# utiasASRL/mm_masking

Measured on AMD Instinct MI355X. Metric: scan-pairs/s (mask-CNN + 10-iter dICP fwd+bwd), higher is better.
Workload: dtype bf16; 1 GPU; BASELINE configs[2]: train_icp_weights step fwd+bwd, batch=32 per GPU, 10 dICP iters, point-to-plane Huber, dim=2; 400x3360 polar radar -> GO-CFAR + peaks + polar->Cartesian 640x640 -> U-Net (hand-written NHWC bf16 MFMA kernels, fp32 masters) -> dICP (fp32 points, fp64 normal equations) -> rot+trans+mask_pts loss -> Adam; batch_per_gpu=32, global_batch=32, scan_pts_pad=5120, map_pts=20000, map_pts_pad=20480, icp_iters=10, parallelism=dp1, scene_density=survey (SURVEY.md 8d: 3 500-5 000 valid scan points of 5 120)

## Files before the change

### include/mmk.h

```cpp
#ifndef MMK_H_
#define MMK_H_

#include <stddef.h>
#include <stdint.h>

#ifdef __cplusplus
extern "C" {
#endif

#define MMK_VERSION 502

#define MMK_OK 0
#define MMK_ERR_ARG (-1)
#define MMK_ERR_HIP (-2)
#define MMK_ERR_WORKSPACE (-3)

#define MMK_ICP_PT2PT 0
#define MMK_ICP_PT2PL 1

#define MMK_NN_BRUTE 0
#define MMK_NN_GRID 1

#define MMK_LOSS_NONE 0
#define MMK_LOSS_CAUCHY 1
// ... 167 lines not shown
                              const float *grad_out, float *grad_x, void *stream);


int mmk_cfar_mask(const float *raw, int32_t B, int32_t A, int32_t R, int32_t w2,
                  int32_t guard, int32_t mincol, int32_t maxcol, float a_thresh,
                  float b_thresh, int32_t diff, float steep_fact, float *mask,
                  void *stream);

int mmk_cfar_mask_bwd(const float *raw, const float *grad_mask , int32_t B, int32_t A, int32_t R, int32_t w2,
                      int32_t guard, int32_t mincol, int32_t maxcol, float a_thresh, float b_thresh, float steep_fact,
                      float *grad_raw , void *stream);

int mmk_cfar_mask_p(const float *raw, int32_t B, int32_t A, int32_t R, int32_t w2, int32_t guard, int32_t mincol,
                    int32_t maxcol, const float *a_thresh, const float *b_thresh, int32_t per_scan, int32_t diff,
                    float steep_fact, float *mask, void *stream);

size_t mmk_cfar_mask_bwd_p_ws_bytes(int32_t B, int32_t A);
int mmk_cfar_mask_bwd_p(const float *raw, const float *grad_mask , int32_t B, int32_t A, int32_t R, int32_t w2,
                        int32_t guard, int32_t mincol, int32_t maxcol, const float *a_thresh, const float *b_thresh,
                        int32_t per_scan, float steep_fact, float *grad_raw , float *grad_a,
                        float *grad_b , void *workspace, size_t workspace_bytes, void *stream);

size_t mmk_extract_peaks_workspace_bytes(int32_t B, int32_t A, int32_t R, int32_t max_pts);
int mmk_extract_peaks(const float *mask, int32_t B, int32_t A, int32_t R, float res,
                      const float *azimuths , const float *times ,
                      const float *T_ab, int32_t diff, float steep_fact, int32_t max_pts,
                      float *out_pc, int32_t *out_count, void *workspace,
                      size_t workspace_bytes, void *stream);
int mmk_extract_peaks_t(const float *mask, int32_t B, int32_t A, int32_t R, float res,
                        const float *azimuths , const float *times ,
                        const float *T_ab, int32_t diff, float steep_fact, int32_t max_pts,
                        float *out_pc, int32_t *out_count, void *workspace,
                        size_t workspace_bytes, float *out_time , void *stream);
size_t mmk_extract_peaks_bwd_workspace_bytes(int32_t B, int32_t A, int32_t R, int32_t max_pts);
int mmk_extract_peaks_bwd(const float *mask, int32_t B, int32_t A, int32_t R, float res, const float *azimuths ,
                          const float *T_ab, int32_t diff, float steep_fact, int32_t max_pts,
                          const float *grad_pc , float *grad_mask , void *workspace,
                          size_t workspace_bytes, void *stream);

int mmk_deskew_points(const float *pc , const float *t , const float *twist ,
                      int32_t B, int32_t N, float *out , void *stream);
size_t mmk_deskew_points_bwd_workspace_bytes(int32_t B, int32_t N);
int mmk_deskew_points_bwd(const float *pc , const float *t , const float *twist ,
                          int32_t B, int32_t N, const float *grad_out ,
                          float *grad_pc , float *grad_twist ,
                          void *workspace, size_t workspace_bytes, void *stream);

int mmk_polar_to_cart(const float *polar, const float *azimuths ,
                      const float *range_grid, const float *angle_grid, int32_t B,
                      int32_t A, int32_t R, int32_t W, float radar_resolution,
                      int32_t interpolate_crossover, int32_t fix_wobble, float *cart,
                      void *stream);
int mmk_polar_to_cart_pair(const float *polar, const float *polar2, const float *azimuths,
                           const float *range_grid, const float *angle_grid, int32_t B, int32_t A,
                           int32_t R, int32_t W, float radar_resolution, int32_t interpolate_crossover,
                           int32_t fix_wobble, float *cart, float *cart2, void *stream);

int mmk_cart_to_polar(const double *cart, const double *sin_az, const double *cos_az, const double *range_coords,
                      int32_t B, int32_t A, int32_t R, int32_t H, int32_t W, double cart_resolution, double *polar,
                      void *stream);

size_t mmk_polar_to_cart_bwd_ws_bytes(int32_t B, int32_t A, int32_t R, int32_t W);
int mmk_polar_to_cart_bwd(const float *grad_cart , const float *azimuths , const float *range_grid,
                          const float *angle_grid, int32_t B, int32_t A, int32_t R, int32_t W, float radar_resolution,
                          int32_t interpolate_crossover, int32_t fix_wobble, float *grad_polar , void *ws,
                          size_t ws_bytes, void *stream);
// ... 200 lines not shown
```

### mm_masking_amd/csrc/mmk_radar.hip

```cpp
#include <math.h>

#include "mmk_common.h"

namespace {

constexpr int RT = 256;

template <int NTHR = RT>
__device__ __forceinline__ double block_excl_scan(double v, double *sm, double *total)
{
    const int lane = threadIdx.x & 63, wv = threadIdx.x >> 6;
    double inc = v;
#pragma unroll
    for (int off = 1; off < 64; off <<= 1) {
        double o = __shfl_up(inc, off, 64);
        if (lane >= off) inc += o;
    }
    if (lane == 63) sm[wv] = inc;
    __syncthreads();
    double base = 0.0, tot = 0.0;
#pragma unroll
    for (int w = 0; w < NTHR / 64; ++w) {
        if (w < wv) base += sm[w];
        tot += sm[w];
    }
    __syncthreads();
    *total = tot;
    return base + inc - v;
}

__device__ __forceinline__ int block_excl_scan_i(int v, int *sm, int *total)
{
    const int lane = threadIdx.x & 63, wv = threadIdx.x >> 6;
    int inc = v;
#pragma unroll
    for (int off = 1; off < 64; off <<= 1) {
        int o = __shfl_up(inc, off, 64);
        if (lane >= off) inc += o;
    }
    if (lane == 63) sm[wv] = inc;
    __syncthreads();
    int base = 0, tot = 0;
#pragma unroll
    for (int w = 0; w < RT / 64; ++w) {
        if (w < wv) base += sm[w];
        tot += sm[w];
    }
    __syncthreads();
    *total = tot;
    return base + inc - v;
}

constexpr int CFAR_T = 512;

struct CfarThVal {
    static constexpr bool per_row = false, params = false;
    float a, b;
    __device__ __forceinline__ int scan_of(int) const { return 0; }
    __device__ __forceinline__ float a_of(int) const { return a; }
    __device__ __forceinline__ float b_of(int) const { return b; }
};
struct CfarThPtr {
    static constexpr bool per_row = true, params = true;
    const float *a, *b;
    int stride, A;
    double *part;
    __device__ __forceinline__ int scan_of(int row) const { return row / A; }
    __device__ __forceinline__ float a_of(int scan) const { return a[scan * stride]; }
    __device__ __forceinline__ float b_of(int scan) const { return b[scan * stride]; }
};

template <class TH>
__global__ __launch_bounds__(CFAR_T) void cfar_mask_kernel(const float *__restrict__ raw, int R, int w2, int guard,
                                                       int mincol, int maxcol, TH thr, int diff,
                                                       float steep, float *__restrict__ mask)
{
    const float a_th = thr.a_of(blockIdx.y), b_th = thr.b_of(blockIdx.y);
    extern __shared__ __attribute__((aligned(16))) unsigned char smem[];
    double *cs = reinterpret_cast<double *>(smem);
    float *row = reinterpret_cast<float *>(cs + (R + 1));
    __shared__ double wsum[CFAR_T / 64];
// ... 168 lines not shown
    }
    if (threadIdx.x == 0) total[b] = tot;
}

__global__ __launch_bounds__(RT) void peaks_emit_kernel(const float *__restrict__ mask, int R, float res, int diff,
                                                        float steep, const int32_t *__restrict__ row_off, int cap,
                                                        float *__restrict__ mval, int32_t *__restrict__ mrow_out)
{
    extern __shared__ __attribute__((aligned(16))) float lrow_dyn[];
    __shared__ int sm[RT / 64];
    const int a = blockIdx.x, b = blockIdx.y, A = gridDim.x;
    const int rowid = b * A + a;
    const float *mrow = stage_row(mask + (size_t)rowid * R, R, lrow_dyn);
    const int L = (R - 1 + RT - 1) / RT;
    const int j0 = min(R - 1, (int)threadIdx.x * L), j1 = min(R - 1, j0 + L);
    int cnt = 0;
    for (int j = j0; j < j1; ++j) cnt += (peak_value(mrow, j, R, res, diff, steep) != 0.0f) ? 1 : 0;
    int tot;
    int g = row_off[rowid] + block_excl_scan_i(cnt, sm, &tot);
    if (cnt != 0) {
        for (int j = j0; j < j1; ++j) {
            const float v = peak_value(mrow, j, R, res, diff, steep);
            if (v != 0.0f) {
                if (g < cap) {
                    mval[(size_t)b * cap + g] = v;
                    mrow_out[(size_t)b * cap + g] = a;
                }
                ++g;
            }
        }
    }
}

__global__ void peaks_pair_kernel(const float *__restrict__ mval, const int32_t *__restrict__ mrow, int cap,
                                  const int32_t *__restrict__ total, const float *__restrict__ az,
                                  const float *__restrict__ T_ab, int A, int max_pts, float *__restrict__ out_pc,
                                  int32_t *__restrict__ out_count)
{
    const int k = blockIdx.x * blockDim.x + threadIdx.x;
    const int b = blockIdx.y;
    const int npts = total[b] / 2;
    if (k == 0) out_count[b] = npts;
    if (k >= max_pts) return;
    float x = 0.f, y = 0.f, z = 0.f;
    if (k < npts && 2 * k + 1 < cap) {
        const size_t m = (size_t)b * cap + 2 * k;
        const float rho = (mval[m + 1] + mval[m]) / 2.0f;
        const float phi = (az[b * A + mrow[m + 1]] + az[b * A + mrow[m]]) / 2.0f;
        x = rho * cosf(phi);
        y = rho * sinf(phi);
        if (T_ab) {
            const float *T = T_ab + (size_t)b * 16;
            const float xx = ((T[0] * x + T[1] * y) + T[2] * z) + T[3];
            const float yy = ((T[4] * x + T[5] * y) + T[6] * z) + T[7];
            const float zz = ((T[8] * x + T[9] * y) + T[10] * z) + T[11];
            x = xx; y = yy; z = zz;
        }
    }
    float *o = out_pc + ((size_t)b * max_pts + k) * 3;
    o[0] = x; o[1] = y; o[2] = z;
}

__global__ void peaks_time_kernel(const int32_t *__restrict__ mrow, int cap, const int32_t *__restrict__ total,
                                  const float *__restrict__ times, int A, int max_pts, float *__restrict__ out_time)
{
    const int k = blockIdx.x * blockDim.x + threadIdx.x;
    const int b = blockIdx.y;
    if (k >= max_pts) return;
    const int npts = total[b] / 2;
    float tv = 0.f;
    if (k < npts && 2 * k + 1 < cap) {
        const size_t m = (size_t)b * cap + 2 * k;
        tv = (times[b * A + mrow[m + 1]] + times[b * A + mrow[m]]) / 2.0f;
    }
    out_time[(size_t)b * max_pts + k] = tv;
}

struct D3 {
    double x, y, z;
};
__device__ __forceinline__ D3 cross3(const D3 &a, const D3 &b) { return {a.y * b.z - a.z * b.y, a.z * b.x - a.x * b.z, a.x * b.y - a.y * b.x}; }
__device__ __forceinline__ double dot3(const D3 &a, const D3 &b) { return (a.x * b.x + a.y * b.y) + a.z * b.z; }
__device__ __forceinline__ D3 scale3(double s, const D3 &a) { return {s * a.x, s * a.y, s * a.z}; }
__device__ __forceinline__ D3 add3(const D3 &a, const D3 &b) { return {a.x + b.x, a.y + b.y, a.z + b.z}; }

constexpr double DESKEW_SERIES_CUT = 1e-4;
constexpr int DESKEW_T = 256;

template <bool WITH_D>
__device__ __forceinline__ void deskew_coef(double th2, double &A, double &B, double &C, double &dA, double &dB, double &dC)
{
    if (th2 < DESKEW_SERIES_CUT) {
        const double th4 = th2 * th2, th6 = th4 * th2;
        A = ((1.0 - th2 / 6.0) + th4 / 120.0) - th6 / 5040.0;
        B = ((0.5 - th2 / 24.0) + th4 / 720.0) - th6 / 40320.0;
        C = ((1.0 / 6.0 - th2 / 120.0) + th4 / 5040.0) - th6 / 362880.0;
        if (WITH_D) {
            dA = (-1.0 / 6.0 + th2 / 60.0) - th4 / 1680.0;
            dB = (-1.0 / 24.0 + th2 / 360.0) - th4 / 13440.0;
            dC = (-1.0 / 120.0 + th2 / 2520.0) - th4 / 120960.0;
        }
    } else {
        const double th = sqrt(th2), s = sin(th), c = cos(th);
        A = s / th;
        B = (1.0 - c) / th2;
        C = (th - s) / (th2 * th);
        if (WITH_D) {
            dA = (C - B) * 0.5;
// ... 194 lines not shown
        const float a3 = laz[c3], a2 = laz[c2];
        const float df = ang - a3;
        const float delta = ((df * ((df < 0.f) ? 1.f : 0.f)) * ((c3 > 0) ? 1.f : 0.f)) / ((a3 - a2) + 1e-14f);
        v = (float)c3 + delta;
        dv = (df < 0.f && c3 > 0) ? 1.0f / ((a3 - a2) + 1e-14f) : 0.f;
    } else {
        const float step = (laz[A - 1] - laz[0]) / (float)(A - 1);
        v = (ang - laz[0]) / step;
        dv = 1.0f / step;
    }
    if (u < 0.f) u = 0.f;
    const int rows = wrap ? A + 2 : A;
    if (wrap) v = v + 1.0f;
    const float gx = u / (float)(R - 1) * 2.0f - 1.0f;
    const float gy = v / (float)(rows - 1) * 2.0f - 1.0f;
    const float ix = ((gx + 1.0f) / 2.0f) * (float)(R - 1);
    const float iy = ((gy + 1.0f) / 2.0f) * (float)(rows - 1);
    const float x0 = floorf(ix), y0 = floorf(iy);
    PolarTaps t;
    t.wx = ix - x0;
    t.wy = iy - y0;
    t.xi = (int)x0;
    t.yi = (int)y0;
    return t;
}

__device__ __forceinline__ PolarTaps polar_taps(const float *laz, float rng, float ang, int A, int R, float res, float half_res,
                                                int wrap, int fix_wobble)
{
    float du, dv;
    return polar_taps_slopes(laz, rng, ang, A, R, res, half_res, wrap, fix_wobble, du, dv);
}

__global__ __launch_bounds__(256) void polar_to_cart_kernel(const float *__restrict__ polar,
                                                            const float *__restrict__ az,
                                                            const float *__restrict__ rgrid,
                                                            const float *__restrict__ agrid, int A, int R, int W,
                                                            float res, float half_res, int wrap, int fix_wobble,
                                                            float *__restrict__ cart, const float *__restrict__ polar2,
                                                            float *__restrict__ cart2)
{
    extern __shared__ float laz[];
    const int b = blockIdx.y;
    for (int i = threadIdx.x; i < A; i += blockDim.x) laz[i] = az[(size_t)b * A + i];
    __syncthreads();
    const int tiles_x = (W + 31) >> 5;
    const int px = (blockIdx.x % tiles_x) * 32 + (threadIdx.x & 31), py = (blockIdx.x / tiles_x) * 8 + (threadIdx.x >> 5);
    if (px >= W || py >= W) return;
    const int pix = py * W + px;
    const int rows = wrap ? A + 2 : A;
    const PolarTaps t = polar_taps(laz, rgrid[pix], agrid[pix], A, R, res, half_res, wrap, fix_wobble);
    const int xi = t.xi, yi = t.yi;
    const float wx = t.wx, wy = t.wy;
    const float ex = 1.0f - wx, sy = 1.0f - wy;
    typedef float f32x2u __attribute__((ext_vector_type(2), aligned(4)));
    const int xa = min(max(xi, 0), R - 2);
    const bool shifted = xi > xa;
    int roff[2];
    bool okr[2];
#pragma unroll
    for (int k = 0; k < 2; ++k) {
        const int yk = yi + k;
        okr[k] = !(yk < 0 || yk >= rows);
        int r = yk;
        if (wrap) r = (yk == 0) ? (A - 1) : ((yk == A + 1) ? 0 : yk - 1);
        roff[k] = min(max(r, 0), A - 1) * R + xa;
    }
    const bool okx0 = xi >= 0 && xi < R, okx1 = xi + 1 >= 0 && xi + 1 < R;
    const float *img = polar + (size_t)b * A * R;
    const float *img2 = polar2 != nullptr ? polar2 + (size_t)b * A * R : img;
    f32x2u p1[2], p2[2];
#pragma unroll
    for (int k = 0; k < 2; ++k) p1[k] = *reinterpret_cast<const f32x2u *>(img + roff[k]);
#pragma unroll
    for (int k = 0; k < 2; ++k) p2[k] = *reinterpret_cast<const f32x2u *>(img2 + roff[k]);
    float t1[4], t2[4];
#pragma unroll
    for (int k = 0; k < 2; ++k) {
        t1[2 * k] = (okr[k] && okx0) ? (shifted ? p1[k].y : p1[k].x) : 0.0f;
        t1[2 * k + 1] = (okr[k] && okx1) ? p1[k].y : 0.0f;
        t2[2 * k] = (okr[k] && okx0) ? (shifted ? p2[k].y : p2[k].x) : 0.0f;
        t2[2 * k + 1] = (okr[k] && okx1) ? p2[k].y : 0.0f;
    }
    cart[(size_t)b * W * W + pix] = t1[0] * (sy * ex) + t1[1] * (sy * wx) + t1[2] * (wy * ex) + t1[3] * (wy * wx);
    if (polar2 != nullptr) cart2[(size_t)b * W * W + pix] = t2[0] * (sy * ex) + t2[1] * (sy * wx) + t2[2] * (wy * ex) + t2[3] * (wy * wx);
}

struct Taps {
    int xi, yi;
    float w00, w01, w10, w11;
    float wx, wy;
};

__device__ __forceinline__ Taps weight_taps(const float *__restrict__ p, int H, int W, int cw, float cres)
{
    const float x = p[0], y = p[1];
    const bool fake = (x == 0.0f) && (y == 0.0f);
    const float gu = -x / cres;
    const float gv = y / cres;
    float gx = gv / (float)(cw - 1) * 2.0f;
    float gy = gu / (float)(cw - 1) * 2.0f;
    if (fake) {
        gx = -100.0f;
        gy = -100.0f;
    }
    const float ix = ((gx + 1.0f) / 2.0f) * (float)(W - 1);
    const float iy = ((gy + 1.0f) / 2.0f) * (float)(H - 1);
    const float x0 = floorf(ix), y0 = floorf(iy);
    const float wx = ix - x0, wy = iy - y0;
    Taps t;
    t.xi = (int)x0;
    t.yi = (int)y0;
    t.w00 = (1.0f - wy) * (1.0f - wx);
    t.w01 = (1.0f - wy) * wx;
    t.w10 = wy * (1.0f - wx);
    t.w11 = wy * wx;
    t.wx = wx;
    t.wy = wy;
// ... 929 lines not shown
    if (int rc = check_workspace(who, workspace, workspace_bytes, w.bytes)) return rc;
    hipStream_t st = (hipStream_t)stream;
    if (int rc = launch_peaks_placement(who, mask, B, A, R, res, diff, steep_fact, w, st)) return rc;
    hipLaunchKernelGGL(peaks_pair_kernel, dim3((max_pts + 255) / 256, B), dim3(256), 0, st, w.mval, w.mrow, w.cap,
                       w.total, azimuths, T_ab, A, max_pts, out_pc, out_count);
    MMK_LAUNCH_CHECK();
    if (out_time) {
        hipLaunchKernelGGL(peaks_time_kernel, dim3((max_pts + 255) / 256, B), dim3(256), 0, st, w.mrow, w.cap, w.total, times, A,
                           max_pts, out_time);
        MMK_LAUNCH_CHECK();
    }
    return MMK_OK;
}

extern "C" int mmk_extract_peaks(const float *mask, int32_t B, int32_t A, int32_t R, float res, const float *azimuths,
                                 const float *times, const float *T_ab, int32_t diff, float steep_fact,
                                 int32_t max_pts, float *out_pc, int32_t *out_count, void *workspace,
                                 size_t workspace_bytes, void *stream)
{
    return run_extract_peaks("mmk_extract_peaks", mask, B, A, R, res, azimuths, times, T_ab, diff, steep_fact, max_pts, out_pc,
                             out_count, workspace, workspace_bytes, nullptr, stream);
}

extern "C" int mmk_extract_peaks_t(const float *mask, int32_t B, int32_t A, int32_t R, float res, const float *azimuths,
                                   const float *times, const float *T_ab, int32_t diff, float steep_fact,
                                   int32_t max_pts, float *out_pc, int32_t *out_count, void *workspace,
                                   size_t workspace_bytes, float *out_time, void *stream)
{
    MMK_REQUIRE(times && out_time, "mmk_extract_peaks_t: NULL times or out_time");
    return run_extract_peaks("mmk_extract_peaks_t", mask, B, A, R, res, azimuths, times, T_ab, diff, steep_fact, max_pts, out_pc,
                             out_count, workspace, workspace_bytes, out_time, stream);
}

static int deskew_args(const char *who, const float *pc, const float *t, const float *twist, int32_t B, int32_t N)
{
    MMK_REQUIRE(pc && t && twist, "%s: NULL pointer", who);
    MMK_REQUIRE(B >= 1 && B <= 65535 && N >= 1, "%s: bad shape (B=%d in 1..65535, N=%d >= 1)", who, B, N);
    return MMK_OK;
}

extern "C" int mmk_deskew_points(const float *pc, const float *t, const float *twist, int32_t B, int32_t N, float *out,
                                 void *stream)
{
    if (int rc = deskew_args("mmk_deskew_points", pc, t, twist, B, N)) return rc;
    MMK_REQUIRE(out, "mmk_deskew_points: NULL pointer");
    hipLaunchKernelGGL(deskew_points_kernel, dim3((N + DESKEW_T - 1) / DESKEW_T, B), dim3(DESKEW_T), 0, (hipStream_t)stream, pc, t,
                       twist, N, out);
    MMK_LAUNCH_CHECK();
    return MMK_OK;
}

extern "C" size_t mmk_deskew_points_bwd_workspace_bytes(int32_t B, int32_t N)
{
    if (B < 1 || N < 1) return 0;
    return mmk::align_up((size_t)B * ((N + DESKEW_T - 1) / DESKEW_T) * 6 * sizeof(double), 256);
}

extern "C" int mmk_deskew_points_bwd(const float *pc, const float *t, const float *twist, int32_t B, int32_t N,
                                     const float *grad_out, float *grad_pc, float *grad_twist, void *workspace,
                                     size_t workspace_bytes, void *stream)
{
    if (int rc = deskew_args("mmk_deskew_points_bwd", pc, t, twist, B, N)) return rc;
    MMK_REQUIRE(grad_out, "mmk_deskew_points_bwd: NULL pointer");
    MMK_REQUIRE(grad_pc || grad_twist, "mmk_deskew_points_bwd: neither gradient is asked for");
    double *part = nullptr;
    if (grad_twist) {
// ... 30 lines not shown
}

extern "C" int mmk_extract_peaks_bwd(const float *mask, int32_t B, int32_t A, int32_t R, float res, const float *azimuths,
                                     const float *T_ab, int32_t diff, float steep_fact, int32_t max_pts, const float *grad_pc,
                                     float *grad_mask, void *workspace, size_t workspace_bytes, void *stream)
{
    MMK_REQUIRE(mask && azimuths && grad_pc && grad_mask, "mmk_extract_peaks_bwd: NULL pointer");
    MMK_REQUIRE(B >= 1 && A >= 1 && R >= 2 && max_pts >= 1, "mmk_extract_peaks_bwd: bad shape");
    const PeakBwdWs w = carve_peaks_bwd(B, A, max_pts, workspace, workspace_bytes);
    if (int rc = check_workspace("mmk_extract_peaks_bwd", workspace, workspace_bytes, w.bytes)) return rc;
    hipStream_t st = (hipStream_t)stream;
    if (int rc = launch_peaks_placement("mmk_extract_peaks_bwd", mask, B, A, R, res, diff, steep_fact, w.f, st)) return rc;
    hipLaunchKernelGGL(peaks_bwd_points_kernel, dim3((max_pts + 255) / 256, B), dim3(256), 0, st, w.f.mrow, w.f.cap, w.f.total,
                       azimuths, T_ab, A, max_pts, grad_pc, w.gv);
    MMK_LAUNCH_CHECK();
    const size_t row_lds = (size_t)R * sizeof(float);
    if (2 * row_lds > 64 * 1024)
        MMK_CHECK_HIP(hipFuncSetAttribute((const void *)peaks_bwd_rows_kernel, hipFuncAttributeMaxDynamicSharedMemorySize,
                                          (int)(2 * row_lds)));
    hipLaunchKernelGGL(peaks_bwd_rows_kernel, dim3(A, B), dim3(RT), 2 * row_lds, st, mask, R, res, diff, steep_fact, w.f.row_off,
                       w.f.cap, w.gv, grad_mask);
    MMK_LAUNCH_CHECK();
    return MMK_OK;
}

static int launch_polar_to_cart(const char *who, const float *polar, const float *polar2, const float *azimuths,
                                const float *range_grid, const float *angle_grid, int32_t B, int32_t A, int32_t R, int32_t W,
                                float radar_resolution, int32_t interpolate_crossover, int32_t fix_wobble, float *cart, float *cart2,
                                void *stream)
{
    MMK_REQUIRE(B >= 1 && A >= 2 && R >= 2 && W >= 1, "%s: bad shape", who);
    MMK_REQUIRE((size_t)A * 4 <= 64 * 1024, "%s: too many azimuths (%d)", who, A);
    const float half_res = (float)((double)radar_resolution / 2.0);
    hipLaunchKernelGGL(polar_to_cart_kernel, dim3(((W + 31) / 32) * ((W + 7) / 8), B), dim3(256), (size_t)A * 4, (hipStream_t)stream,
                       polar, azimuths, range_grid, angle_grid, A, R, W, radar_resolution, half_res,
                       interpolate_crossover ? 1 : 0, fix_wobble ? 1 : 0, cart, polar2, cart2);
    MMK_LAUNCH_CHECK();
    return MMK_OK;
}

extern "C" int mmk_polar_to_cart(const float *polar, const float *azimuths, const float *range_grid,
                                 const float *angle_grid, int32_t B, int32_t A, int32_t R, int32_t W,
                                 float radar_resolution, int32_t interpolate_crossover, int32_t fix_wobble, float *cart,
                                 void *stream)
{
    MMK_REQUIRE(polar && azimuths && range_grid && angle_grid && cart, "mmk_polar_to_cart: NULL pointer");
    return launch_polar_to_cart("mmk_polar_to_cart", polar, nullptr, azimuths, range_grid, angle_grid, B, A, R, W, radar_resolution,
                                interpolate_crossover, fix_wobble, cart, nullptr, stream);
}

extern "C" int mmk_polar_to_cart_pair(const float *polar, const float *polar2, const float *azimuths, const float *range_grid,
                                      const float *angle_grid, int32_t B, int32_t A, int32_t R, int32_t W,
                                      float radar_resolution, int32_t interpolate_crossover, int32_t fix_wobble, float *cart,
                                      float *cart2, void *stream)
{
    MMK_REQUIRE(polar && polar2 && azimuths && range_grid && angle_grid && cart && cart2, "mmk_polar_to_cart_pair: NULL pointer");
    return launch_polar_to_cart("mmk_polar_to_cart_pair", polar, polar2, azimuths, range_grid, angle_grid, B, A, R, W,
                                radar_resolution, interpolate_crossover, fix_wobble, cart, cart2, stream);
}

extern "C" int mmk_cart_to_polar(const double *cart, const double *sin_az, const double *cos_az, const double *range_coords,
                                 int32_t B, int32_t A, int32_t R, int32_t H, int32_t W, double cart_resolution, double *polar,
                                 void *stream)
{
    MMK_REQUIRE(cart && sin_az && cos_az && range_coords && polar, "mmk_cart_to_polar: NULL pointer");
    MMK_REQUIRE(B >= 1 && B <= 65535 && A >= 1 && A <= 65535 && R >= 1 && H >= 2 && W >= 2, "mmk_cart_to_polar: bad shape");
    MMK_REQUIRE(cart_resolution > 0.0, "mmk_cart_to_polar: cart_resolution must be positive");
// ... 313 lines not shown
```

### mm_masking_amd/radar_utils.py

```python
import ctypes

import numpy as np
import torch

from . import _lib

__all__ = ["load_pc_from_file", "load_radar", "cfar_mask", "extract_pc", "extract_pc_padded", "extract_weights",
           "extract_weights_polar", "polar_target_from_pts", "extract_bev_from_pts", "mean_peaks_parallel_fast", "pol_2_cart", "radar_polar_to_cartesian",
           "radar_polar_to_cartesian_diff", "radar_cartesian_to_polar", "mask_polar_scan", "point_to_cart_idx",
           "form_cart_range_angle_grid", "form_polar_range_grid", "scan_times", "deskew_pc"]


def _hip_device(t):
    if t.is_cuda:
        return t.device
    if not torch.cuda.is_available():
        raise _lib.MmkError("radar_utils needs an MI355X/HIP device: the operators are HIP kernels with no CPU path")
    return torch.device("cuda", torch.cuda.current_device())


def _back(out, like):
    return out if like.is_cuda else out.to(like.device)


def _sized_workspace(size_fn, device, *dims):
    return _lib.workspace(int(size_fn(*dims)), device, "radar")


def _remember(ctx, *inputs):
    ctx.like = [(t.dtype, t.device, tuple(t.shape)) if torch.is_tensor(t) else None for t in inputs]


def _grads_back(ctx, grads, n_rest):
    return tuple(None if g is None else g.to(device=like[1], dtype=like[0]) for g, like in zip(grads, ctx.like)) + (None,) * n_rest


def load_pc_from_file(file_path, to_type=None, to_device="cpu"):
    pc = np.fromfile(file_path, dtype=np.float32)
    pc = torch.from_numpy(pc.reshape((len(pc) // 6, 6))).to(to_device)
    return pc if to_type is None else pc.type(to_type)
# ... 322 lines not shown
        _remember(ctx, thres_mask)
        ctx.mark_non_differentiable(*out[1:])
        return out

    @staticmethod
    def backward(ctx, gpc, *_rest):
        m, az, Tab = ctx.saved_tensors
        res, diff, steep_fact, max_pts = ctx.args
        B, A, R = m.shape
        dev = m.device
        gpc = _lib.dev_f32(gpc, dev)
        L = _lib.lib()
        ws = _sized_workspace(L.mmk_extract_peaks_bwd_workspace_bytes, dev, B, A, R, max_pts)
        gm = torch.empty_like(m)
        _lib.check(L.mmk_extract_peaks_bwd(_lib.ptr(m), B, A, R, res, _lib.ptr(az), _lib.ptr(Tab), diff, steep_fact, max_pts,
                                           _lib.ptr(gpc), _lib.ptr(gm), _lib.ptr(ws), ws.numel(), _lib.stream_ptr(dev)))
        return _grads_back(ctx, (gm,), 9)


def extract_pc_padded(thres_mask, res, azimuth_angles, azimuth_times, max_pts, T_ab=None, diff=True,
                      steep_fact=10.0, return_times=False):
    if return_times and azimuth_times is None:
        raise ValueError("extract_pc_padded: return_times=True needs azimuth_times")
    dev = _hip_device(thres_mask)
    m = _lib.dev_f32(thres_mask, dev)
    az = _lib.dev_f32(azimuth_angles, dev)
    tm = _lib.dev_f32(azimuth_times, dev) if azimuth_times is not None else None
    Tab = _lib.dev_f32(T_ab, dev).reshape(-1, 16) if T_ab is not None else None
    if torch.is_grad_enabled() and thres_mask.requires_grad:
        return _ExtractPeaks.apply(thres_mask, m, res, az, tm, Tab, diff, steep_fact, max_pts, bool(return_times))
    return _peaks_forward(m, res, az, tm, Tab, diff, steep_fact, max_pts, bool(return_times))


def scan_times(az_times, unit=1e-6, ref="mid"):
    if ref not in ("mid", "first", "last"):
        raise ValueError("scan_times: ref must be 'mid', 'first' or 'last' (got %r)" % (ref,))
    if az_times.ndim != 2:
        raise ValueError("scan_times: az_times must be (B, A) (got %s)" % (tuple(az_times.shape),))
    t = az_times.detach().to(torch.float64)
    lo, hi = t.amin(dim=1, keepdim=True), t.amax(dim=1, keepdim=True)
    t0 = lo if ref == "first" else hi if ref == "last" else lo + (hi - lo) / 2
    return ((t - t0) * float(unit)).to(torch.float32)


class _DeskewPoints(torch.autograd.Function):

    @staticmethod
    def forward(ctx, pc, twist, dev, t):
        p, w = _lib.dev_f32(pc, dev), _lib.dev_f32(twist, dev)
        out = _deskew_forward(p, t, w)
        ctx.save_for_backward(p, t, w)
        _remember(ctx, pc, twist)
        return _back(out, pc)

    @staticmethod
    def backward(ctx, g):
        p, t, w = ctx.saved_tensors
        B, N = t.shape
        dev = p.device
        g = _lib.dev_f32(g, dev)
        want_pc, want_twist = ctx.needs_input_grad[0], ctx.needs_input_grad[1]
        L = _lib.lib()
        ws = _sized_workspace(L.mmk_deskew_points_bwd_workspace_bytes, dev, B, N) if want_twist else None
        gp = torch.empty_like(p) if want_pc else None
        gw = torch.empty_like(w) if want_twist else None
        _lib.check(L.mmk_deskew_points_bwd(_lib.ptr(p), _lib.ptr(t), _lib.ptr(w), B, N, _lib.ptr(g), _lib.ptr(gp), _lib.ptr(gw),
# ... 243 lines not shown
```

### mm_masking_amd/train_icp_weights.py

```python
import time

import torch

from . import _lib
from . import radar_utils as ru
from . import synthetic
from .icp_weight_policy import LearnICPWeightPolicy, _check_batch


def default_params(device=None):
    if device is None:
        device = torch.device("cuda" if torch.cuda.is_available() else "cpu")
    return {
        "device": device, "float_type": torch.float32, "gt_eye": True, "pos_std": 2.0, "rot_std": 0.6,
        "z_std": 0.0, "tilt_std": 0.0, "pose_loss": "se2",
        "log_transform": False, "normalize": ["minmax"], "batch_size_train": 16, "batch_size_test": 32,
        "icp_type": "pt2pt", "learning_rate": 1e-4, "leaky": False, "dropout": 0.05, "batch_norm": False,
        "init_weights": True, "a_thresh": 1.0, "b_thresh": 0.09, "loss_icp_rot_weight": 1.0,
        "loss_icp_trans_weight": 1.0, "loss_fft_mask_weight": 0.0, "loss_map_pts_mask_weight": 1.0,
        "loss_cfar_mask_weight": 0.0, "num_pts_weight": 0.0, "optimizer": "adam", "icp_loss_only_iter": -1,
        "max_iter": 10, "network_input_type": "cartesian", "network_output_type": "cartesian",
        "binary_inference": False, "norm_weights": True, "fft_input": True, "cfar_input": False,
        "range_input": False, "num_epochs": 30,
    }


def loss_weights_from(params):
    return {"icp_rot": params["loss_icp_rot_weight"], "icp_trans": params["loss_icp_trans_weight"],
            "fft": params["loss_fft_mask_weight"], "mask_pts": params["loss_map_pts_mask_weight"],
            "cfar": params["loss_cfar_mask_weight"], "num_pts": params["num_pts_weight"]}


def prepare_batch(raw, params, max_loc_pts=5120, polar_res=0.0596):
    motion = bool(params.get("motion_comp", False))
    if motion and (raw.get("velocity") is None or raw.get("az_times") is None):
        raise ValueError("motion_comp needs raw['velocity'] (B,6) and raw['az_times'] (synthetic.make_pair with vel_std or "
                         "yawrate_std > 0)")
    fft = raw["fft_polar"]
    az = raw["azimuths"]
    cfar = ru.cfar_mask(fft, polar_res, a_thresh=params["a_thresh"], b_thresh=params["b_thresh"], diff=False)
    if motion:
        seconds = ru.scan_times(raw["az_times"], params.get("motion_time_unit", 1e-6), params.get("motion_ref", "mid"))
        pc, _, t = ru.extract_pc_padded(cfar, polar_res, az, seconds, max_loc_pts, diff=False, return_times=True)
        filtered = ru.deskew_pc(pc, t, raw["velocity"])
    else:
        pc, _ = ru.extract_pc_padded(cfar, polar_res, az, raw["az_times"], max_loc_pts, diff=False)
        filtered = pc
    if params.get("network_input_type", "cartesian") == "cartesian":
        fft_img, cfar_img = ru._polar_to_cart_pair(fft, cfar, az, polar_res)
    else:
        fft_img, cfar_img = fft, cfar
    loc_data = {"raw_pc": pc, "filtered_pc": filtered, "fft_data": fft_img, "fft_cfar": cfar_img, "timestamp": 0}
    if motion:
        loc_data["velocity"] = raw["velocity"]
    if params.get("mask_target") == "scan":
        loc_data.update({"fft_polar": fft, "azimuths": az, "az_times": raw["az_times"]})
    if params.get("polar_sampling"):
        loc_data["azimuths"] = az
    map_data = {"pc": raw["map_pc"], "timestamp": 0}
    T_data = {"T_ml_init": raw["T_init"], "T_ml_gt": raw["T_gt"]}
    return {"loc_data": loc_data, "map_data": map_data, "transforms": T_data}


_CONST_CACHE = {}


def _const(kind, device, dtype):
    key = (kind, device, dtype)
    t = _CONST_CACHE.get(key)
    if t is None:
        t = torch.zeros(1, dtype=dtype, device=device) if kind == "zero" else torch.eye(4, dtype=dtype, device=device)
        _CONST_CACHE[key] = t
    return t


def _on_hip_f32(*tensors):
    return all(t.is_cuda and t.dtype == torch.float32 for t in tensors)


# ... 491 lines not shown
```

Baseline: 3465 pairs/s.

## Fuse CFAR mask and peak extraction into persistent row kernel plus pair kernel

Adds a front-end path where a persistent CFAR kernel computes the mask per row, prefetches the next row, and writes per-row peak counts and values into a workspace slab. A second kernel prefix-sums the row counts, finds each point pair by binary search and emits points and times, replacing the separate CFAR, placement, pair and time launches. The aim is fewer launches and less re-reading of the mask. Polar-to-Cartesian blocks now also process four tiles each. Rows with more peaks than the slab holds fall back to a slow serial walk of the mask.

```diff
diff --git a/include/mmk.h b/include/mmk.h
--- a/include/mmk.h
+++ b/include/mmk.h
@@ -223,6 +223,12 @@
                         const float *T_ab, int32_t diff, float steep_fact, int32_t max_pts,
                         float *out_pc, int32_t *out_count, void *workspace,
                         size_t workspace_bytes, float *out_time , void *stream);
+size_t mmk_scan_front_end_workspace_bytes(int32_t B, int32_t A, int32_t R, int32_t max_pts, int32_t row_cap);
+int mmk_scan_front_end(const float *raw, int32_t B, int32_t A, int32_t R, int32_t w2, int32_t guard, int32_t mincol,
+                       int32_t maxcol, float a_thresh, float b_thresh, int32_t diff, float steep_fact, float res,
+                       const float *azimuths , const float *times , const float *T_ab, int32_t max_pts,
+                       int32_t row_cap, float *mask , float *out_pc , int32_t *out_count ,
+                       float *out_time , void *workspace, size_t workspace_bytes, void *stream);
 size_t mmk_extract_peaks_bwd_workspace_bytes(int32_t B, int32_t A, int32_t R, int32_t max_pts);
 int mmk_extract_peaks_bwd(const float *mask, int32_t B, int32_t A, int32_t R, float res, const float *azimuths ,
                           const float *T_ab, int32_t diff, float steep_fact, int32_t max_pts,
diff --git a/mm_masking_amd/csrc/mmk_radar.hip b/mm_masking_amd/csrc/mmk_radar.hip
--- a/mm_masking_amd/csrc/mmk_radar.hip
+++ b/mm_masking_amd/csrc/mmk_radar.hip
@@ -29,6 +29,7 @@
     return base + inc - v;
 }
 
+template <int NTHR = RT, bool TRAIL = true>
 __device__ __forceinline__ int block_excl_scan_i(int v, int *sm, int *total)
 {
     const int lane = threadIdx.x & 63, wv = threadIdx.x >> 6;
@@ -42,11 +43,11 @@
     __syncthreads();
     int base = 0, tot = 0;
 #pragma unroll
-    for (int w = 0; w < RT / 64; ++w) {
+    for (int w = 0; w < NTHR / 64; ++w) {
         if (w < wv) base += sm[w];
         tot += sm[w];
     }
-    __syncthreads();
+    if (TRAIL) __syncthreads();
     *total = tot;
     return base + inc - v;
 }
@@ -281,6 +282,22 @@
     }
 }
 
+__device__ __forceinline__ void pair_point(float v0, float v1, float az0, float az1, const float *__restrict__ T, float &x, float &y,
+                                           float &z)
+{
+    const float rho = (v1 + v0) / 2.0f;
+    const float phi = (az1 + az0) / 2.0f;
+    x = rho * cosf(phi);
+    y = rho * sinf(phi);
+    z = 0.f;
+    if (T) {
+        const float xx = ((T[0] * x + T[1] * y) + T[2] * z) + T[3];
+        const float yy = ((T[4] * x + T[5] * y) + T[6] * z) + T[7];
+        const float zz = ((T[8] * x + T[9] * y) + T[10] * z) + T[11];
+        x = xx; y = yy; z = zz;
+    }
+}
+
 __global__ void peaks_pair_kernel(const float *__restrict__ mval, const int32_t *__restrict__ mrow, int cap,
                                   const int32_t *__restrict__ total, const float *__restrict__ az,
                                   const float *__restrict__ T_ab, int A, int max_pts, float *__restrict__ out_pc,
@@ -294,17 +311,7 @@
     float x = 0.f, y = 0.f, z = 0.f;
     if (k < npts && 2 * k + 1 < cap) {
         const size_t m = (size_t)b * cap + 2 * k;
-        const float rho = (mval[m + 1] + mval[m]) / 2.0f;
-        const float phi = (az[b * A + mrow[m + 1]] + az[b * A + mrow[m]]) / 2.0f;
-        x = rho * cosf(phi);
-        y = rho * sinf(phi);
-        if (T_ab) {
-            const float *T = T_ab + (size_t)b * 16;
-            const float xx = ((T[0] * x + T[1] * y) + T[2] * z) + T[3];
-            const float yy = ((T[4] * x + T[5] * y) + T[6] * z) + T[7];
-            const float zz = ((T[8] * x + T[9] * y) + T[10] * z) + T[11];
-            x = xx; y = yy; z = zz;
-        }
+        pair_point(mval[m], mval[m + 1], az[b * A + mrow[m]], az[b * A + mrow[m + 1]], T_ab ? T_ab + (size_t)b * 16 : nullptr, x, y, z);
     }
     float *o = out_pc + ((size_t)b * max_pts + k) * 3;
     o[0] = x; o[1] = y; o[2] = z;
@@ -323,6 +330,171 @@
         tv = (times[b * A + mrow[m + 1]] + times[b * A + mrow[m]]) / 2.0f;
     }
     out_time[(size_t)b * max_pts + k] = tv;
+}
+
+template <int NPRE, class TH>
+__global__ __launch_bounds__(CFAR_T) void cfar_peaks_rows_kernel(const float *__restrict__ raw, int rows, int R, int w2, int guard,
+                                                                 int mincol, int maxcol, TH thr, int diff, float steep, float res,
+                                                                 int row_cap, float *__restrict__ mask,
+                                                                 int32_t *__restrict__ row_count, float *__restrict__ slab)
+{
+    extern __shared__ __attribute__((aligned(16))) unsigned char smem[];
+    double *cs = reinterpret_cast<double *>(smem);
+    float *row = reinterpret_cast<float *>(cs + (R + 1));
+    __shared__ double wsum[CFAR_T / 64];
+    float nx[NPRE];
+    int r = blockIdx.x;
+    if (r >= rows) return;
+    auto fetch = [&](int rr) {
+        const float *src = raw + (size_t)rr * R;
+#pragma unroll
+        for (int i = 0; i < NPRE; ++i) {
+            const int c = threadIdx.x + i * CFAR_T;
+            nx[i] = src[c < R ? c : R - 1];
+        }
+    };
+    auto stage = [&]() {
+#pragma unroll
+        for (int i = 0; i < NPRE; ++i) {
+            const int c = threadIdx.x + i * CFAR_T;
+            if (c < R) row[c] = nx[i];
+        }
+    };
+    fetch(r);
+    stage();
+    __syncthreads();
+    const int L = (R + CFAR_T - 1) / CFAR_T;
+    const int c0 = min(R, (int)threadIdx.x * L), c1 = min(R, c0 + L);
+    const int LP = (R - 1 + CFAR_T - 1) / CFAR_T;
+    const int j0 = min(R - 1, (int)threadIdx.x * LP), j1 = min(R - 1, j0 + LP);
+    float a_th = thr.a_of(thr.scan_of(r)), b_th = thr.b_of(thr.scan_of(r));
+    while (true) {
+        const int rn = r + gridDim.x;
+        fetch(rn < rows ? rn : r);
+        double s = 0.0;
+        for (int c = c0; c < c1; ++c) s += (double)row[c];
+        double tot;
+        double run = block_excl_scan<CFAR_T>(s, wsum, &tot);
+        for (int c = c0; c < c1; ++c) {
+            cs[c] = run;
+            run += (double)row[c];
+        }
+        if (threadIdx.x == CFAR_T - 1) cs[R] = tot;
+        __syncthreads();
+        float *out = mask + (size_t)r * R;
+        for (int c = threadIdx.x; c < R; c += CFAR_T) {
+            float th = 1000.0f;
+            if (c >= mincol && c < maxcol) {
+                const float left = (float)(cs[c - guard] - cs[c - w2 - guard]);
+                const float right = (float)(cs[min(R, c + w2 + guard + 1)] - cs[min(R, c + guard + 1)]);
+                const float stat = fmaxf(left, right) / (float)w2;
+                th = a_th * stat + b_th;
+            }
+            const float x = row[c];
+            float m;
+            if (diff) {
+                m = 0.5f * tanhf(steep * (x - th) + 2.5f) + 0.5f;
+                m = (fabsf(m) > 0.99f) ? m : 0.0f;
+            } else {
+                m = (x > th) ? 1.0f : 0.0f;
+            }
+            out[c] = m;
+            row[c] = m;
+        }
+        __syncthreads();
+        int cnt = 0;
+        for (int j = j0; j < j1; ++j) cnt += (peak_value(row, j, R, res, diff, steep) != 0.0f) ? 1 : 0;
+        int ntot;
+        int pos = block_excl_scan_i<CFAR_T, false>(cnt, reinterpret_cast<int *>(wsum), &ntot);
+        if (threadIdx.x == 0) row_count[r] = ntot;
+        if (cnt != 0) {
+            float *dst = slab + (size_t)r * row_cap;
+            for (int j = j0; j < j1; ++j) {
+                const float v = peak_value(row, j, R, res, diff, steep);
+                if (v != 0.0f) {
+                    if (pos < row_cap) dst[pos] = v;
+                    ++pos;
+                }
+            }
+        }
+        if (rn >= rows) break;
+        __syncthreads();
+        stage();
+        __syncthreads();
+        r = rn;
+        if (TH::per_row) {
+            a_th = thr.a_of(thr.scan_of(r));
+            b_th = thr.b_of(thr.scan_of(r));
+        }
+    }
+}
+
+__device__ __forceinline__ float marker_by_walk(const float *__restrict__ mrow, int pos, int R, float res, int diff, float steep)
+{
+    int seen = 0;
+    for (int j = 0; j < R - 1; ++j) {
+        const float v = peak_value(mrow, j, R, res, diff, steep);
+        if (v != 0.0f) {
+            if (seen == pos) return v;
+            ++seen;
+        }
+    }
+    return 0.0f;
+}
+
+__global__ __launch_bounds__(RT) void peaks_pair_rows_kernel(const int32_t *__restrict__ row_count, const float *__restrict__ slab,
+                                                             int row_cap, const float *__restrict__ mask, int R, float res, int diff,
+                                                             float steep, const float *__restrict__ az,
+                                                             const float *__restrict__ times, const float *__restrict__ T_ab, int A,
+                                                             int max_pts, int32_t *__restrict__ total, float *__restrict__ out_pc,
+                                                             int32_t *__restrict__ out_count, float *__restrict__ out_time)
+{
+    extern __shared__ __attribute__((aligned(16))) int off_dyn[];
+    __shared__ int sm[RT / 64];
+    const int b = blockIdx.y;
+    const int32_t *rc = row_count + (size_t)b * A;
+    const int L = (A + RT - 1) / RT;
+    const int a0 = min(A, (int)threadIdx.x * L), a1 = min(A, a0 + L);
+    int s = 0;
+    for (int a = a0; a < a1; ++a) s += rc[a];
+    int tot;
+    int run = block_excl_scan_i(s, sm, &tot);
+    for (int a = a0; a < a1; ++a) {
+        off_dyn[a] = run;
+        run += rc[a];
+    }
+    if (threadIdx.x == 0) off_dyn[A] = tot;
+    __syncthreads();
+    const int k = blockIdx.x * RT + threadIdx.x;
+    const int npts = tot / 2;
+    if (k == 0) {
+        total[b] = tot;
+        out_count[b] = npts;
+    }
+    if (k >= max_pts) return;
+    float x = 0.f, y = 0.f, z = 0.f, tv = 0.f;
+    if (k < npts) {
+        float v[2];
+        int ar[2];
+#pragma unroll
+        for (int i = 0; i < 2; ++i) {
+            const int m = 2 * k + i;
+            int lo = 0, hi = A - 1;
+            while (lo < hi) {
+                const int mid = (lo + hi + 1) >> 1;
+                if (off_dyn[mid] <= m) lo = mid; else hi = mid - 1;
+            }
+            const int pos = m - off_dyn[lo];
+            const size_t rowid = (size_t)b * A + lo;
+            v[i] = (pos < row_cap) ? slab[rowid * row_cap + pos] : marker_by_walk(mask + rowid * R, pos, R, res, diff, steep);
+            ar[i] = lo;
+        }
+        pair_point(v[0], v[1], az[b * A + ar[0]], az[b * A + ar[1]], T_ab ? T_ab + (size_t)b * 16 : nullptr, x, y, z);
+        if (out_time) tv = (times[b * A + ar[1]] + times[b * A + ar[0]]) / 2.0f;
+    }
+    float *o = out_pc + ((size_t)b * max_pts + k) * 3;
+    o[0] = x; o[1] = y; o[2] = z;
+    if (out_time) out_time[(size_t)b * max_pts + k] = tv;
 }
 
 struct D3 {
@@ -583,6 +755,7 @@
     return polar_taps_slopes(laz, rng, ang, A, R, res, half_res, wrap, fix_wobble, du, dv);
 }
 
+constexpr int P2C_TILES = 4;
 __global__ __launch_bounds__(256) void polar_to_cart_kernel(const float *__restrict__ polar,
                                                             const float *__restrict__ az,
                                                             const float *__restrict__ rgrid,
@@ -596,45 +769,48 @@
     for (int i = threadIdx.x; i < A; i += blockDim.x) laz[i] = az[(size_t)b * A + i];
     __syncthreads();
     const int tiles_x = (W + 31) >> 5;
-    const int px = (blockIdx.x % tiles_x) * 32 + (threadIdx.x & 31), py = (blockIdx.x / tiles_x) * 8 + (threadIdx.x >> 5);
-    if (px >= W || py >= W) return;
-    const int pix = py * W + px;
+    const int n_tiles = tiles_x * ((W + 7) >> 3);
     const int rows = wrap ? A + 2 : A;
-    const PolarTaps t = polar_taps(laz, rgrid[pix], agrid[pix], A, R, res, half_res, wrap, fix_wobble);
-    const int xi = t.xi, yi = t.yi;
-    const float wx = t.wx, wy = t.wy;
-    const float ex = 1.0f - wx, sy = 1.0f - wy;
-    typedef float f32x2u __attribute__((ext_vector_type(2), aligned(4)));
-    const int xa = min(max(xi, 0), R - 2);
-    const bool shifted = xi > xa;
-    int roff[2];
-    bool okr[2];
-#pragma unroll
-    for (int k = 0; k < 2; ++k) {
-        const int yk = yi + k;
-        okr[k] = !(yk < 0 || yk >= rows);
-        int r = yk;
-        if (wrap) r = (yk == 0) ? (A - 1) : ((yk == A + 1) ? 0 : yk - 1);
-        roff[k] = min(max(r, 0), A - 1) * R + xa;
-    }
-    const bool okx0 = xi >= 0 && xi < R, okx1 = xi + 1 >= 0 && xi + 1 < R;
-    const float *img = polar + (size_t)b * A * R;
-    const float *img2 = polar2 != nullptr ? polar2 + (size_t)b * A * R : img;
-    f32x2u p1[2], p2[2];
-#pragma unroll
-    for (int k = 0; k < 2; ++k) p1[k] = *reinterpret_cast<const f32x2u *>(img + roff[k]);
-#pragma unroll
-    for (int k = 0; k < 2; ++k) p2[k] = *reinterpret_cast<const f32x2u *>(img2 + roff[k]);
-    float t1[4], t2[4];
-#pragma unroll
-    for (int k = 0; k < 2; ++k) {
-        t1[2 * k] = (okr[k] && okx0) ? (shifted ? p1[k].y : p1[k].x) : 0.0f;
-        t1[2 * k + 1] = (okr[k] && okx1) ? p1[k].y : 0.0f;
-        t2[2 * k] = (okr[k] && okx0) ? (shifted ? p2[k].y : p2[k].x) : 0.0f;
-        t2[2 * k + 1] = (okr[k] && okx1) ? p2[k].y : 0.0f;
-    }
-    cart[(size_t)b * W * W + pix] = t1[0] * (sy * ex) + t1[1] * (sy * wx) + t1[2] * (wy * ex) + t1[3] * (wy * wx);
-    if (polar2 != nullptr) cart2[(size_t)b * W * W + pix] = t2[0] * (sy * ex) + t2[1] * (sy * wx) + t2[2] * (wy * ex) + t2[3] * (wy * wx);
+    for (int tile = blockIdx.x * P2C_TILES; tile < min(n_tiles, ((int)blockIdx.x + 1) * P2C_TILES); ++tile) {
+        const int px = (tile % tiles_x) * 32 + (threadIdx.x & 31), py = (tile / tiles_x) * 8 + (threadIdx.x >> 5);
+        if (px >= W || py >= W) continue;
+        const int pix = py * W + px;
+        const PolarTaps t = polar_taps(laz, rgrid[pix], agrid[pix], A, R, res, half_res, wrap, fix_wobble);
+        const int xi = t.xi, yi = t.yi;
+        const float wx = t.wx, wy = t.wy;
+        const float ex = 1.0f - wx, sy = 1.0f - wy;
+        typedef float f32x2u __attribute__((ext_vector_type(2), aligned(4)));
+        const int xa = min(max(xi, 0), R - 2);
+        const bool shifted = xi > xa;
+        int roff[2];
+        bool okr[2];
+#pragma unroll
+        for (int k = 0; k < 2; ++k) {
+            const int yk = yi + k;
+            okr[k] = !(yk < 0 || yk >= rows);
+            int r = yk;
+            if (wrap) r = (yk == 0) ? (A - 1) : ((yk == A + 1) ? 0 : yk - 1);
+            roff[k] = min(max(r, 0), A - 1) * R + xa;
+        }
+        const bool okx0 = xi >= 0 && xi < R, okx1 = xi + 1 >= 0 && xi + 1 < R;
+        const float *img = polar + (size_t)b * A * R;
+        const float *img2 = polar2 != nullptr ? polar2 + (size_t)b * A * R : img;
+        f32x2u p1[2], p2[2];
+#pragma unroll
+        for (int k = 0; k < 2; ++k) p1[k] = *reinterpret_cast<const f32x2u *>(img + roff[k]);
+#pragma unroll
+        for (int k = 0; k < 2; ++k) p2[k] = *reinterpret_cast<const f32x2u *>(img2 + roff[k]);
+        float t1[4], t2[4];
+#pragma unroll
+        for (int k = 0; k < 2; ++k) {
+            t1[2 * k] = (okr[k] && okx0) ? (shifted ? p1[k].y : p1[k].x) : 0.0f;
+            t1[2 * k + 1] = (okr[k] && okx1) ? p1[k].y : 0.0f;
+            t2[2 * k] = (okr[k] && okx0) ? (shifted ? p2[k].y : p2[k].x) : 0.0f;
+            t2[2 * k + 1] = (okr[k] && okx1) ? p2[k].y : 0.0f;
+        }
+        cart[(size_t)b * W * W + pix] = t1[0] * (sy * ex) + t1[1] * (sy * wx) + t1[2] * (wy * ex) + t1[3] * (wy * wx);
+        if (polar2 != nullptr) cart2[(size_t)b * W * W + pix] = t2[0] * (sy * ex) + t2[1] * (sy * wx) + t2[2] * (wy * ex) + t2[3] * (wy * wx);
+    }
 }
 
 struct Taps {
@@ -1630,6 +1806,90 @@
                              out_count, workspace, workspace_bytes, out_time, stream);
 }
 
+constexpr int FRONT_ROW_CAP = 256;
+constexpr size_t PAIR_OFF_LDS_MAX = 64 * 1024 - 64;
+
+struct FrontWs {
+    int32_t *row_count, *total;
+    float *slab;
+    size_t bytes;
+};
+
+static FrontWs carve_front(int B, int A, int row_cap, void *ws, size_t cap_bytes)
+{
+    mmk::Arena ar(ws, cap_bytes);
+    FrontWs w;
+    w.row_count = ar.take<int32_t>((size_t)B * A);
+    w.total = ar.take<int32_t>((size_t)B);
+    w.slab = ar.take<float>((size_t)B * A * row_cap);
+    w.bytes = mmk::align_up(ar.off, 256);
+    return w;
+}
+
+static bool front_end_fused(int32_t A, int32_t R)
+{
+    const size_t smem = (size_t)(R + 1) * sizeof(double) + (size_t)R * sizeof(float);
+    return R <= 8 * CFAR_T && smem <= 40 * 1024 && ((size_t)A + 1) * sizeof(int) <= PAIR_OFF_LDS_MAX;
+}
+
+extern "C" size_t mmk_scan_front_end_workspace_bytes(int32_t B, int32_t A, int32_t R, int32_t max_pts, int32_t row_cap)
+{
+    if (B < 1 || A < 1 || R < 2 || max_pts < 1) return 0;
+    if (row_cap <= 0) row_cap = FRONT_ROW_CAP;
+    return std::max(carve_front(B, A, row_cap, nullptr, 0).bytes, carve_peaks(B, A, max_pts, nullptr, 0).bytes);
+}
+
+extern "C" int mmk_scan_front_end(const float *raw, int32_t B, int32_t A, int32_t R, int32_t w2, int32_t guard, int32_t mincol,
+                                  int32_t maxcol, float a_thresh, float b_thresh, int32_t diff, float steep_fact, float res,
+                                  const float *azimuths, const float *times, const float *T_ab, int32_t max_pts, int32_t row_cap,
+                                  float *mask, float *out_pc, int32_t *out_count, float *out_time, void *workspace,
+                                  size_t workspace_bytes, void *stream)
+{
+    const char *who = "mmk_scan_front_end";
+    MMK_REQUIRE(raw && mask && azimuths && out_pc && out_count, "%s: NULL pointer", who);
+    MMK_REQUIRE(!out_time || times, "%s: out_time needs times", who);
+    CfarCall c{raw, B, A, R, w2, guard, mincol, maxcol, steep_fact, (hipStream_t)stream, 0};
+    if (int rc = cfar_args(who, c)) return rc;
+    MMK_REQUIRE(R >= 2 && max_pts >= 1, "%s: bad shape", who);
+    if (row_cap <= 0) row_cap = FRONT_ROW_CAP;
+    if (int rc = check_workspace(who, workspace, workspace_bytes, mmk_scan_front_end_workspace_bytes(B, A, R, max_pts, row_cap))) return rc;
+    const dim3 pair_grid((max_pts + 255) / 256, B);
+    if (!front_end_fused(A, R)) {
+        if (int rc = launch_cfar_fwd(c, CfarThVal{a_thresh, b_thresh}, diff, mask)) return rc;
+        const PeakWs w = carve_peaks(B, A, max_pts, workspace, workspace_bytes);
+        if (int rc = launch_peaks_placement(who, mask, B, A, R, res, diff, steep_fact, w, c.st)) return rc;
+        hipLaunchKernelGGL(peaks_pair_kernel, pair_grid, dim3(256), 0, c.st, w.mval, w.mrow, w.cap, w.total, azimuths, T_ab, A, max_pts,
+                           out_pc, out_count);
+        MMK_LAUNCH_CHECK();
+        if (out_time) {
+            hipLaunchKernelGGL(peaks_time_kernel, pair_grid, dim3(256), 0, c.st, w.mrow, w.cap, w.total, times, A, max_pts, out_time);
+            MMK_LAUNCH_CHECK();
+        }
+        return MMK_OK;
+    }
+    const FrontWs w = carve_front(B, A, row_cap, workspace, workspace_bytes);
+    const int rows = A * B;
+    int dev = 0, cus = 256;
+    if (hipGetDevice(&dev) == hipSuccess) {
+        int v = 0;
+        if (hipDeviceGetAttribute(&v, hipDeviceAttributeMultiprocessorCount, dev) == hipSuccess && v > 0) cus = v;
+    }
+    int per_cu = 0;
+    if (hipOccupancyMaxActiveBlocksPerMultiprocessor(&per_cu, (const void *)(cfar_peaks_rows_kernel<8, CfarThVal>), CFAR_T, c.smem) !=
+            hipSuccess || per_cu < 1 || per_cu > 4) {
+        (void)hipGetLastError();
+        per_cu = 4;
+    }
+    const int grid = std::min(rows, per_cu * cus);
+    hipLaunchKernelGGL((cfar_peaks_rows_kernel<8, CfarThVal>), dim3(grid), dim3(CFAR_T), c.smem, c.st, raw, rows, R, w2, guard, mincol,
+                       maxcol, CfarThVal{a_thresh, b_thresh}, diff, steep_fact, res, row_cap, mask, w.row_count, w.slab);
+    MMK_LAUNCH_CHECK();
+    hipLaunchKernelGGL(peaks_pair_rows_kernel, pair_grid, dim3(RT), ((size_t)A + 1) * sizeof(int), c.st, w.row_count, w.slab, row_cap,
+                       mask, R, res, diff, steep_fact, azimuths, times, T_ab, A, max_pts, w.total, out_pc, out_count, out_time);
+    MMK_LAUNCH_CHECK();
+    return MMK_OK;
+}
+
 static int deskew_args(const char *who, const float *pc, const float *t, const float *twist, int32_t B, int32_t N)
 {
     MMK_REQUIRE(pc && t && twist, "%s: NULL pointer", who);
@@ -1726,7 +1986,7 @@
     MMK_REQUIRE(B >= 1 && A >= 2 && R >= 2 && W >= 1, "%s: bad shape", who);
     MMK_REQUIRE((size_t)A * 4 <= 64 * 1024, "%s: too many azimuths (%d)", who, A);
     const float half_res = (float)((double)radar_resolution / 2.0);
-    hipLaunchKernelGGL(polar_to_cart_kernel, dim3(((W + 31) / 32) * ((W + 7) / 8), B), dim3(256), (size_t)A * 4, (hipStream_t)stream,
+    hipLaunchKernelGGL(polar_to_cart_kernel, dim3((((W + 31) / 32) * ((W + 7) / 8) + P2C_TILES - 1) / P2C_TILES, B), dim3(256), (size_t)A * 4, (hipStream_t)stream,
                        polar, azimuths, range_grid, angle_grid, A, R, W, radar_resolution, half_res,
                        interpolate_crossover ? 1 : 0, fix_wobble ? 1 : 0, cart, polar2, cart2);
     MMK_LAUNCH_CHECK();
diff --git a/mm_masking_amd/radar_utils.py b/mm_masking_amd/radar_utils.py
--- a/mm_masking_amd/radar_utils.py
+++ b/mm_masking_amd/radar_utils.py
@@ -1,11 +1,14 @@
 import ctypes
+import os
 
 import numpy as np
 import torch
 
 from . import _lib
 
-__all__ = ["load_pc_from_file", "load_radar", "cfar_mask", "extract_pc", "extract_pc_padded", "extract_weights",
+FRONT_END_FUSED = os.environ.get("MMK_FRONT_END_FUSED", "1") != "0"
+
+__all__ = ["load_pc_from_file", "load_radar", "cfar_mask", "extract_pc", "extract_pc_padded", "cfar_extract_pc_padded", "extract_weights",
            "extract_weights_polar", "polar_target_from_pts", "extract_bev_from_pts", "mean_peaks_parallel_fast", "pol_2_cart", "radar_polar_to_cartesian",
            "radar_polar_to_cartesian_diff", "radar_cartesian_to_polar", "mask_polar_scan", "point_to_cart_idx",
            "form_cart_range_angle_grid", "form_polar_range_grid", "scan_times", "deskew_pc"]
@@ -394,6 +397,38 @@
     return _peaks_forward(m, res, az, tm, Tab, diff, steep_fact, max_pts, bool(return_times))
 
 
+def cfar_extract_pc_padded(raw_scans, res, azimuth_angles, azimuth_times, max_pts, width=101, minr=2.0, maxr=80.0, guard=5,
+                           a_thresh=1.0, b_thresh=0.09, T_ab=None, diff=True, steep_fact=10.0, return_times=False, row_cap=0):
+    if return_times and azimuth_times is None:
+        raise ValueError("cfar_extract_pc_padded: return_times=True needs azimuth_times")
+    assert raw_scans.ndim == 3, "raw_scans must be 3D"
+    fused = (FRONT_END_FUSED and isinstance(diff, bool) and not torch.is_tensor(a_thresh) and not torch.is_tensor(b_thresh)
+             and not (torch.is_grad_enabled() and raw_scans.requires_grad))
+    if not fused:
+        mask = cfar_mask(raw_scans, res, width, minr, maxr, guard, a_thresh, b_thresh, diff, steep_fact)
+        return (mask,) + tuple(extract_pc_padded(mask, res, azimuth_angles, azimuth_times, max_pts, T_ab=T_ab, diff=diff,
+                                                 steep_fact=steep_fact, return_times=return_times))
+    dev = _hip_device(raw_scans)
+    x = _lib.dev_f32(raw_scans, dev)
+    B, A, R = x.shape
+    w2, mincol, maxcol = cfar_cols(R, res, width, minr, maxr, guard)
+    az = _lib.dev_f32(azimuth_angles, dev)
+    tm = _lib.dev_f32(azimuth_times, dev) if return_times else None
+    Tab = _lib.dev_f32(T_ab, dev).reshape(-1, 16) if T_ab is not None else None
+    L = _lib.lib()
+    ws = _sized_workspace(L.mmk_scan_front_end_workspace_bytes, dev, B, A, R, int(max_pts), int(row_cap))
+    mask = torch.empty_like(x)
+    pc = torch.empty(B, int(max_pts), 3, dtype=torch.float32, device=dev)
+    cnt = torch.empty(B, dtype=torch.int32, device=dev)
+    t = torch.empty(B, int(max_pts), dtype=torch.float32, device=dev) if return_times else None
+    _lib.check(L.mmk_scan_front_end(_lib.ptr(x), B, A, R, w2, guard, mincol, max(mincol, maxcol), float(a_thresh), float(b_thresh),
+                                    1 if diff else 0, float(steep_fact), float(res), _lib.ptr(az), _lib.ptr(tm), _lib.ptr(Tab),
+                                    int(max_pts), int(row_cap), _lib.ptr(mask), _lib.ptr(pc), _lib.ptr(cnt), _lib.ptr(t),
+                                    _lib.ptr(ws), ws.numel(), _lib.stream_ptr(dev)))
+    out = (_back(mask, raw_scans), pc, cnt)
+    return out + (t,) if return_times else out
+
+
 def scan_times(az_times, unit=1e-6, ref="mid"):
     if ref not in ("mid", "first", "last"):
         raise ValueError("scan_times: ref must be 'mid', 'first' or 'last' (got %r)" % (ref,))
diff --git a/mm_masking_amd/train_icp_weights.py b/mm_masking_amd/train_icp_weights.py
--- a/mm_masking_amd/train_icp_weights.py
+++ b/mm_masking_amd/train_icp_weights.py
@@ -38,13 +38,14 @@
                          "yawrate_std > 0)")
     fft = raw["fft_polar"]
     az = raw["azimuths"]
-    cfar = ru.cfar_mask(fft, polar_res, a_thresh=params["a_thresh"], b_thresh=params["b_thresh"], diff=False)
+    thresholds = {"a_thresh": params["a_thresh"], "b_thresh": params["b_thresh"]}
     if motion:
         seconds = ru.scan_times(raw["az_times"], params.get("motion_time_unit", 1e-6), params.get("motion_ref", "mid"))
-        pc, _, t = ru.extract_pc_padded(cfar, polar_res, az, seconds, max_loc_pts, diff=False, return_times=True)
+        cfar, pc, _, t = ru.cfar_extract_pc_padded(fft, polar_res, az, seconds, max_loc_pts, diff=False, return_times=True,
+                                                   **thresholds)
         filtered = ru.deskew_pc(pc, t, raw["velocity"])
     else:
-        pc, _ = ru.extract_pc_padded(cfar, polar_res, az, raw["az_times"], max_loc_pts, diff=False)
+        cfar, pc, _ = ru.cfar_extract_pc_padded(fft, polar_res, az, raw["az_times"], max_loc_pts, diff=False, **thresholds)
         filtered = pc
     if params.get("network_input_type", "cartesian") == "cartesian":
         fft_img, cfar_img = ru._polar_to_cart_pair(fft, cfar, az, polar_res)
```

Measured after the change: 3483 pairs/s (median of 2 runs). Within noise of the previous version (+0.5%).
